# rjzhb/VectorSearch-RBAC

Hardware: AMD Instinct MI355X
Metric: QPS at recall@100, SIFT10M filtered-kNN (role RBAC), 1/2/4/8 MI355X (higher is better)
Workload: dtype int8 planes -> i32 (exact: bit-identical to the fp32 distances of vector.c)

## Files before the change

vectorsearch-rbac_amd/csrc/vsr_device.h:

```cpp
#pragma once
#include <hip/hip_runtime.h>
#include <stdint.h>
#include "vsr_bounds.h"

namespace vsr {

using f32x4 = __attribute__((ext_vector_type(4))) float;
using u32x4 = __attribute__((ext_vector_type(4))) uint32_t;
using i32x4 = __attribute__((ext_vector_type(4))) int;
using bf16x8 = __attribute__((ext_vector_type(8))) __bf16;
using f16x8 = __attribute__((ext_vector_type(8))) _Float16;

#ifdef __HIPCC__
template <class T> using gptr = const __attribute__((address_space(1))) T*;
template <class T> __device__ __forceinline__ gptr<T> as_global(const T* p) { return (gptr<T>) p; }
template <class T> __device__ __forceinline__ T lds_peek(const T* p)
{
    return *(const volatile __attribute__((address_space(3))) T*) p;
}
__device__ __forceinline__ uint2 load_tile(gptr<uint2> tiles, uint32_t t)
{
    const uint64_t v = ((gptr<uint64_t>) tiles)[t];
    return make_uint2((uint32_t) v, (uint32_t) (v >> 32));
}
#endif

constexpr uint64_t KEY_EMPTY = ~0ull;
constexpr int      SCAN_THREADS = 512;
constexpr int      SCAN_WAVES = SCAN_THREADS / 64;
constexpr int      SELECT_THREADS = 1024;
constexpr int      MAX_K = 2048;
constexpr int      SCAN_QMAX = 16;
constexpr size_t   SCAN_LDS_BUDGET = 72 * 1024;

constexpr int scan_slack(int rw) { return SCAN_WAVES * rw > 256 ? SCAN_WAVES * rw : 256; }

enum Metric : int { M_L2 = 0, M_IP = 1, M_COSINE = 2, M_L1 = 3 };

struct ScanGroup {
    const uint2*    tiles;
    const uint64_t* bitmap;
    uint32_t        n_tiles;
    uint32_t        q_begin;
    uint32_t        q_count;
    uint32_t        block_begin;
    uint32_t        n_blocks;
    uint32_t        partial_begin;
};

struct FusedTail {
    uint32_t        enable;
    uint32_t        fan;
    ScanGroup       group;
    uint32_t*       done;
    const int64_t*  block_ids;
    const int32_t*  doc_ids;
    const int64_t*  orig_rows;
    int64_t*        out_block;
    int32_t*        out_doc;
    int64_t*        out_row;
    float*          out_dist;
    uint64_t*       out_keys;
    int32_t*        out_count;
    int32_t*        out_flag;
    int32_t*        flag_total;
    uint32_t        row_offset;
    int             metric;
    uint64_t*       dbg;
};

#ifndef VSR_MW_DENSE
#define VSR_MW_DENSE 1
#endif

struct ScanParams {
    const float4*    rows;
    const float*     norm2;
    uint32_t         n_rows;
    uint32_t         stride4;
    const float*     queries;
    const float*     q_norm2;
    const ScanGroup* groups;
    uint32_t         n_groups;
    const uint32_t*  q_slots;
    uint64_t*        partial;
    uint32_t         kp;
    uint32_t         k;
    uint32_t         cap;
    uint32_t         qmax;
    uint64_t*        cand;
    uint32_t         rw;
    const uint64_t*  tau_init;
    uint32_t         sample_stride;
    const uint2*     block_map;
    const uint4*     scr;
    const uint4*     q_scr;
    uint32_t         pstride4;
    const uint4*     scr_c;
    const uint4*     q_scr_c;
    uint32_t         cstride4;
    uint32_t         plane_ho;
    uint64_t*        qcand;
    uint32_t*        qcnt;
    uint32_t         capq;
    const uint32_t*  rank;
    const uint64_t*  ones;
// ... 280 lines not shown
```

vectorsearch-rbac_amd/csrc/vsr_i8r.h:

```cpp
#pragma once
#include <type_traits>
#include "vsr_device.h"
#include "vsr_topk.h"
#include "vsr_mfma.h"

namespace vsr {

constexpr int KR_THREADS = 256;
constexpr int KR_WAVES = 4;
constexpr int KR_RING = 4;
constexpr int KR_OCC = 5;

template <int NQG>
__global__ __launch_bounds__(KR_THREADS, KR_OCC) void i8_sample_reg_kernel(const ScanParams p)
{
    constexpr int NC = NQG * 16;
    static_assert(NC == 64, "one lane of the appending wave per query column");
    __shared__ __align__(16) uint4 s_b[NQG * 2 * 64];
    __shared__ uint2 s_col[NC];
    static_assert(sizeof(uint4) * NQG * 2 * 64 >= sizeof(uint64_t) * KR_WAVES * NC * 4, "minima do not fit the B area");
    const int tid = threadIdx.x;
    const int lane = tid & 63;
    const int wave = __builtin_amdgcn_readfirstlane(tid >> 6);

    uint32_t lo = 0, hi = p.n_groups;
    while (hi - lo > 1) {
        const uint32_t mid = (lo + hi) >> 1;
        if (p.groups[mid].block_begin <= blockIdx.x) lo = mid; else hi = mid;
    }
    const ScanGroup grp = p.groups[lo];
    const uint32_t local_block = blockIdx.x - grp.block_begin;
    const auto g_tiles = as_global(grp.tiles);
    const auto g_norm2 = as_global(p.norm2);
    const auto g_rank = as_global(p.rank);
    const uint32_t q_count = grp.q_count;

    uint4 bq[2];
#pragma unroll
    for (int e = 0; e < 2; ++e) {
        const uint32_t idx = (uint32_t) tid + 256u * e;
        const uint32_t qi = (idx >> 7) * 16u + (idx & 15u);
        const uint32_t slot = p.q_slots[grp.q_begin + (qi < q_count ? qi : 0u)];
        bq[e] = p.q_scr[(size_t) slot * p.pstride4 + ((idx >> 6) & 1u) * 4u + ((idx & 63u) >> 4)];
    }
    if (tid < NC) {
        const bool qok = (uint32_t) tid < q_count;
        const uint32_t slot = p.q_slots[grp.q_begin + (qok ? (uint32_t) tid : 0u)];
        s_col[tid] = make_uint2(__float_as_uint(p.q_norm2[slot]), qok ? slot : 0xFFFFFFFFu);
    }

    const uint32_t t0 = (uint32_t) (((uint64_t) grp.n_tiles * local_block) / grp.n_blocks);
    const uint32_t t1 = (uint32_t) (((uint64_t) grp.n_tiles * (local_block + 1)) / grp.n_blocks);
    const uint32_t ss = p.sample_stride;
    const uint32_t n_st = (((t1 - t0 + 1u) >> 1) + ss - 1u) / ss;
    const uint32_t n_w = n_st > (uint32_t) wave ? (n_st - (uint32_t) wave + 3u) >> 2 : 0u;
    const uint32_t n_units = 2u * n_w;
    const uint32_t unit_last = n_units ? n_units - 1u : 0u;

    const uint32_t tile_last = grp.n_tiles - 1u;
    uint32_t row_lo, row_hi;
    bool bad_row;
    {
        const uint2 da = load_tile(g_tiles, t0 < tile_last ? t0 : tile_last);
        const uint2 db = load_tile(g_tiles, t1 > t0 && t1 - 1u < tile_last ? t1 - 1u : tile_last);
        row_lo = (uint32_t) __builtin_amdgcn_readfirstlane((int) da.x);
        row_hi = t1 > t0 ? (uint32_t) __builtin_amdgcn_readfirstlane((int) (db.x + db.y)) : row_lo;
        bad_row = row_hi > p.n_rows || row_hi < row_lo;
        row_hi = bad_row ? row_lo : row_hi;
    }
    const uint32_t row_clamp = (p.n_rows - 1u) & ~15u;

    const int li = lane & 15;
    const int kq = lane >> 4;
    const uint32_t ngt = (q_count + 15u) >> 4;
    const uint32_t voff = (uint32_t) li * 128u + (uint32_t) kq * 16u;
    const char* scr = reinterpret_cast<const char*>(p.scr);

    auto unit_row = [&](uint32_t u) -> uint32_t {
        const uint32_t uc = u < unit_last ? u : unit_last;
        return row_lo + 32u * ss * ((uint32_t) wave + 4u * (uc >> 1)) + 16u * (uc & 1u);
    };
    i32x4 a8[KR_RING][2];
    f32x4 nrm[KR_RING];
    auto issue = [&](auto K, uint32_t u) {
        constexpr int k = decltype(K)::value;
        const uint32_t r0 = unit_row(u);
        const uint32_t rc = r0 < row_clamp ? r0 : row_clamp;
        const gptr<uint4> src = as_global(reinterpret_cast<const uint4*>(scr + (size_t) rc * 128u + voff));
        a8[k][0] = __builtin_bit_cast(i32x4, src[0]);
        a8[k][1] = __builtin_bit_cast(i32x4, src[4]);
        nrm[k] = *reinterpret_cast<gptr<f32x4>>(g_norm2 + rc + (uint32_t) kq * 4u);
    };
    issue(std::integral_constant<int, 0>{}, 0u);
    issue(std::integral_constant<int, 1>{}, 1u);
    issue(std::integral_constant<int, 2>{}, 2u);

    s_b[tid] = bq[0];
    s_b[tid + 256] = bq[1];
    asm volatile("s_waitcnt lgkmcnt(0)\n\ts_barrier" ::: "memory");

    int64_t smin[NQG];
#pragma unroll
    for (int j = 0; j < NQG; ++j) smin[j] = ((int64_t) 0x3FFFFFFF << 32);
    auto compute = [&](auto K, uint32_t u) {
        constexpr int k = decltype(K)::value;
        const uint32_t row = unit_row(u) + (uint32_t) kq * 4u;
        int32_t nx[4];
#pragma unroll
        for (int r = 0; r < 4; ++r) nx[r] = row + (uint32_t) r < row_hi ? (int32_t) nrm[k][r] : 0x3FFFFFFF;
#pragma unroll
        for (int j = 0; j < NQG; ++j) {
            if ((uint32_t) j < ngt) {
                const i32x4 b0 = __builtin_bit_cast(i32x4, s_b[(j * 2 + 0) * 64 + lane]);
                const i32x4 b1 = __builtin_bit_cast(i32x4, s_b[(j * 2 + 1) * 64 + lane]);
                i32x4 acc = i32x4{0, 0, 0, 0};
                acc = __builtin_amdgcn_mfma_i32_16x16x64_i8(a8[k][0], b0, acc, 0, 0, 0);
                acc = __builtin_amdgcn_mfma_i32_16x16x64_i8(a8[k][1], b1, acc, 0, 0, 0);
#pragma unroll
                for (int r = 0; r < 4; ++r) {
                    const int32_t w = nx[r] - 2 * acc[r];
                    const int64_t cand = ((int64_t) w << 32) | (int64_t) (row + (uint32_t) r);
                    smin[j] = cand < smin[j] ? cand : smin[j];
                }
            }
        }
    };
    for (uint32_t u = 0; u < n_units; u += 4u) {
        issue(std::integral_constant<int, 3>{}, u + 3u);
        compute(std::integral_constant<int, 0>{}, u);
        issue(std::integral_constant<int, 0>{}, u + 4u);
        compute(std::integral_constant<int, 1>{}, u + 1u);
        issue(std::integral_constant<int, 1>{}, u + 5u);
        compute(std::integral_constant<int, 2>{}, u + 2u);
        issue(std::integral_constant<int, 2>{}, u + 6u);
        compute(std::integral_constant<int, 3>{}, u + 3u);
    }

    asm volatile("s_waitcnt lgkmcnt(0)\n\ts_barrier" ::: "memory");
    uint64_t* keys = reinterpret_cast<uint64_t*>(s_b);
#pragma unroll
    for (int j = 0; j < NQG; ++j) {
        const int32_t w = (int32_t) (smin[j] >> 32);
        uint64_t key = KEY_EMPTY;
        if ((uint32_t) j < ngt && w < 0x20000000) {
            const uint2 cc = s_col[j * 16 + li];
            const uint32_t row = (uint32_t) smin[j];
            if (cc.y != 0xFFFFFFFFu) key = make_key((float) w + __uint_as_float(cc.x), g_rank ? g_rank[row] : row);
        }
        keys[(wave * NC + j * 16 + li) * 4 + kq] = key;
    }
    asm volatile("s_waitcnt lgkmcnt(0)\n\ts_barrier" ::: "memory");
    if (wave == 0) {
        const int c = lane;
        const uint32_t slot = s_col[c].y;
        uint64_t keys16[4 * KR_WAVES];
        uint32_t n = 0;
#pragma unroll
        for (int w2 = 0; w2 < KR_WAVES; ++w2)
#pragma unroll
            for (int q4 = 0; q4 < 4; ++q4) {
                const uint64_t kk = keys[(w2 * NC + c) * 4 + q4];
                keys16[w2 * 4 + q4] = kk;
                n += kk != KEY_EMPTY;
            }
        if (n && slot != 0xFFFFFFFFu) {
            uint32_t at = atomicAdd(p.qcnt + slot, n);
#pragma unroll
            for (int t = 0; t < 4 * KR_WAVES; ++t)
                if (keys16[t] != KEY_EMPTY) {
                    if (at < p.capq) p.qcand[(size_t) slot * p.capq + at] = keys16[t];
                    ++at;
                }
        }
// ... 13 lines not shown
```

vectorsearch-rbac_amd/csrc/vsr_mfmaw.h:

```cpp
#pragma once
#include <type_traits>
#include "vsr_device.h"
#include "vsr_scan.h"
#include "vsr_topk.h"
#include "vsr_mfma.h"
#include "vsr_i8s.h"
#include "vsr_i8r.h"

namespace vsr {

constexpr int MW_THREADS = 256;
constexpr int MW_WAVES = 4;
constexpr int MW_S = 16;
constexpr int MW_ROWS = 64;
constexpr int MW_NQ = MF_NQ * MW_WAVES;
constexpr int MW_RING = 8;

#ifndef VSR_MW_DEPTH1
#define VSR_MW_DEPTH1 1
#endif
#ifndef VSR_MW_OCC1
#define VSR_MW_OCC1 3
#endif
#ifndef VSR_ABLATE
// ... 130 lines not shown
    const uint32_t g1 = (uint32_t) wave + 4u;
    const bool gact2 = NG == 2 && rsplit == 1u && g1 < ngt;
    const uint32_t my_qi2 = g1 * MF_NQ + (uint32_t) jq;
    const bool qok2 = gact2 && my_qi2 < q_count;
    uint32_t my_slot2 = my_slot;
    float my_qn2 = 0.0f, tau_lim2 = -__builtin_inff();
    const uint4* my_qsrc2 = nullptr;
    bf16x8 bh2[NBLK], bm2[NBLK];
    if constexpr (NG == 2) {
        my_slot2 = p.q_slots[grp.q_begin + (qok2 ? my_qi2 : 0u)];
        const uint64_t t2 = p.tau_init ? p.tau_init[my_slot2] : KEY_EMPTY;
        tau_lim2 = t2 == KEY_EMPTY ? __builtin_inff() : mono_to_float((uint32_t) (t2 >> 32));
        my_qn2 = p.q_norm2[my_slot2];
        my_qsrc2 = p.q_scr + (size_t) my_slot2 * (HO ? 2 * pstride4 : pstride4);
#pragma unroll
        for (int blk = 0; blk < NBLK; ++blk) {
            bh2[blk] = __builtin_bit_cast(bf16x8, my_qsrc2[blk * 4 + kq]);
            bm2[blk] = __builtin_bit_cast(bf16x8, my_qsrc2[(HO ? 16 : 8) + blk * 4 + kq]);
        }
    }
    const uint32_t col_slot = lane < MF_NQ ? my_slot : my_slot2;

    const uint32_t tile_last = grp.n_tiles - 1u;
    auto fetch_desc = [&](uint32_t it_) -> uint2 {
        const uint32_t t = t0 + it_ * ss * tps + (uint32_t) lane / rw;
        const bool ok = it_ < n_it && t < t1;
        const uint2 d = load_tile(g_tiles, t < tile_last ? t : tile_last);
        return make_uint2(ok ? d.x : 0u, ok ? d.y : 0u);
    };
    int32_t  pend_row[DEPTH];
    uint64_t pend_bw[DEPTH];
    float    pend_nrm[DEPTH];
    uint2    dsc_a[DEPTH];
#pragma unroll
    for (int j = 0; j < DEPTH; ++j) {
        pend_row[j] = -1;
        pend_bw[j] = ~0ull;
        pend_nrm[j] = 0.0f;
        dsc_a[j] = make_uint2(0u, 0u);
    }
    bool bad_row = false;
    uint32_t row_lo = 0, row_hi = 0;
    if constexpr (DENSE) {
        const uint2 da = load_tile(g_tiles, t0 < tile_last ? t0 : tile_last);
        const uint2 db = load_tile(g_tiles, t1 > t0 && t1 - 1u < tile_last ? t1 - 1u : tile_last);
        row_lo = (uint32_t) __builtin_amdgcn_readfirstlane((int) da.x);
        row_hi = t1 > t0 ? (uint32_t) __builtin_amdgcn_readfirstlane((int) (db.x + db.y)) : row_lo;
        bad_row = row_hi > p.n_rows || row_hi < row_lo;
        row_hi = bad_row ? row_lo : row_hi;
    }
    auto start_dense = [&](uint32_t it_, int32_t& row, uint64_t& bw, float& nrm) {
        const uint32_t rr = row_lo + it_ * (uint32_t) MW_ROWS + (uint32_t) lane;
        const bool ok = it_ < n_it && rr < row_hi;
        row = ok ? (int32_t) rr : -1;
        bw = ~0ull;
        nrm = g_norm2[ok ? rr : 0u];
    };
    auto start_rows = [&](uint2 d, int32_t& row, uint64_t& bw, float& nrm) {
        const uint32_t r = (uint32_t) lane % rw;
        const uint32_t rr = d.x + r;
        const bool ok = r < d.y && rr < p.n_rows;
        bad_row |= r < d.y && rr >= p.n_rows;
        const uint32_t rc = ok ? rr : 0u;
        row = ok ? (int32_t) rr : -1;
        bw = *(g_bitmap ? g_bitmap + (rc >> 6) : g_ones);
        nrm = g_norm2[rc];
    };
    auto finish_rows = [&](uint32_t it_, int32_t row, uint64_t bw, float nrm) {
        if (row >= 0 && !((bw >> ((uint32_t) row & 63u)) & 1ull)) row = -1;
        if (wave == 0) {
            rowidx[(it_ % MW_RING) * 64 + lane] = row;
            rownorm[(it_ % MW_RING) * 64 + lane] = row >= 0 ? nrm : __builtin_nanf("");
            if constexpr (ITEST) rowthr[(it_ % MW_RING) * 64 + lane] = row >= 0 ? ((int32_t) nrm) >> 1 : 0x7FFFFFFF;
        }
    };
    if constexpr (DENSE) {
#pragma unroll
        for (int j = 0; j < DEPTH; ++j) {
            int32_t r0;
            uint64_t b0;
            float n0;
            start_dense((uint32_t) j, r0, b0, n0);
            finish_rows((uint32_t) j, r0, b0, n0);
            start_dense((uint32_t) (DEPTH + j), pend_row[j], pend_bw[j], pend_nrm[j]);
        }
    } else {
        uint2 d[2 * DEPTH];
#pragma unroll
        for (int j = 0; j < 2 * DEPTH; ++j) d[j] = fetch_desc((uint32_t) j);
#pragma unroll
        for (int j = 0; j < DEPTH; ++j) dsc_a[j] = fetch_desc((uint32_t) (2 * DEPTH + j));
#pragma unroll
        for (int j = 0; j < DEPTH; ++j) {
            int32_t r0;
            uint64_t b0;
            float n0;
            start_rows(d[j], r0, b0, n0);
            finish_rows((uint32_t) j, r0, b0, n0);
            start_rows(d[DEPTH + j], pend_row[j], pend_bw[j], pend_nrm[j]);
        }
    }
    __syncthreads();

    const int lrow = I8 ? tid >> 3 : tid >> 4, lchunk = I8 ? tid & 7 : tid & 15;
    constexpr int LROWS = I8 ? 32 : 16;
    uint4 X[DEPTH][NCHR][NU];
    const uint32_t last_row = p.n_rows - 1u;
    auto issue = [&](auto dc, auto sc, uint32_t it_) {
        constexpr int D = decltype(dc)::value;
        constexpr int S = decltype(sc)::value;
        const uint32_t chunk = (uint32_t) (S * SR + lchunk);
        const int32_t* ridx = rowidx + (it_ % MW_RING) * 64;
#pragma unroll
        for (int u = 0; u < NU; ++u) {
            uint32_t rc;
            if constexpr (DENSE) {
                const uint32_t rr = row_lo + it_ * (uint32_t) MW_ROWS + (uint32_t) (u * LROWS + lrow);
                rc = it_ < n_it && rr < row_hi ? rr : 0u;
            } else {
                const int32_t r = ridx[u * LROWS + lrow];
                rc = (uint32_t) (r < 0 ? 0 : r);
            }
            if ((VSR_ABLATE & 8) && it_ > 0) continue;
            const u32x4 v = *reinterpret_cast<const u32x4*>(p.scr + (size_t) (rc < last_row ? rc : last_row) * pstride4 + chunk);
            X[D][S][u] = make_uint4(v[0], v[1], v[2], v[3]);
        }
    };
    const uint32_t nch_rt = LONG ? pstride4 / (uint32_t) SR : (uint32_t) NCH;
    auto issue_rt = [&](uint32_t it_, uint32_t s_) {
        const uint32_t chunk = s_ * (uint32_t) SR + (uint32_t) lchunk;
        const int32_t* ridx = rowidx + (it_ % MW_RING) * 64;
#pragma unroll
        for (int u = 0; u < NU; ++u) {
            const int32_t r = ridx[u * LROWS + lrow];
            const uint32_t rc = (uint32_t) (r < 0 ? 0 : r);
            const u32x4 v = *reinterpret_cast<const u32x4*>(p.scr + (size_t) (rc < last_row ? rc : last_row) * pstride4 + chunk);
            X[0][0][u] = make_uint4(v[0], v[1], v[2], v[3]);
        }
    };
    auto load_b = [&](uint32_t s_, bf16x8 (&h)[NBLK], bf16x8 (&m)[NBLK]) {
#pragma unroll
        for (int blk = 0; blk < NBLK; ++blk) {
            h[blk] = __builtin_bit_cast(bf16x8, my_qsrc[s_ * (HO ? 32u : 16u) + (uint32_t) (blk * 4 + kq)]);
            m[blk] = __builtin_bit_cast(bf16x8, my_qsrc[s_ * (HO ? 32u : 16u) + (HO ? 16u : 8u) + (uint32_t) (blk * 4 + kq)]);
        }
    };
    auto issue_tile = [&](auto dc, uint32_t it_) {
        if constexpr (LONG) {
            issue_rt(it_, 0u);
            return;
        }
        issue(dc, std::integral_constant<int, 0>{}, it_);
        if constexpr (NCH > 1) issue(dc, std::integral_constant<int, 1>{}, it_);
        if constexpr (NCH > 2) issue(dc, std::integral_constant<int, 2>{}, it_);
    };
    const uint32_t n_pad = (n_it + DEPTH - 1) / DEPTH * DEPTH;
    issue_tile(std::integral_constant<int, 0>{}, 0);
    if constexpr (DEPTH > 1) issue_tile(std::integral_constant<int, 1>{}, 1);
    if constexpr (DEPTH > 2) issue_tile(std::integral_constant<int, 2>{}, 2);
    if constexpr (DEPTH > 3) issue_tile(std::integral_constant<int, 3>{}, 3);

    uint32_t p_head = 0, p_tail = 0, f_n = 0;
    constexpr int FL_R = 2;
    uint32_t f_rank[FL_R];
    uint32_t f_base = 0;
#pragma unroll
    for (int r = 0; r < FL_R; ++r) f_rank[r] = 0;
    auto flush_issue = [&]() __attribute__((always_inline)) {
        const uint32_t have = p_tail - p_head;
        f_n = have < 64u * FL_R ? have : 64u * FL_R;
        uint32_t col[FL_R];
#pragma unroll
        for (int r = 0; r < FL_R; ++r) {
            const uint32_t e = (uint32_t) (r * 64 + lane);
            col[r] = e < f_n ? pend_c[(p_head + e) % MW_PEND] : 0xFFu;
        }
        uint32_t mine = 0;
#pragma unroll
        for (int c = 0; c < MF_NQ * NG; ++c) {
            uint32_t before = 0;
#pragma unroll
            for (int r = 0; r < FL_R; ++r) {
                const uint64_t m = __ballot(col[r] == (uint32_t) c);
                if (col[r] == (uint32_t) c)
                    f_rank[r] = before + __builtin_amdgcn_mbcnt_hi((uint32_t) (m >> 32), __builtin_amdgcn_mbcnt_lo((uint32_t) m, 0u));
                before += (uint32_t) __popcll(m);
            }
            if (lane == c) mine = before;
        }
        if (lane < MF_NQ * NG && mine) f_base = atomicAdd(p.qcnt + col_slot, mine);
    };
    auto flush_store = [&]() __attribute__((always_inline)) {
#pragma unroll
        for (int r = 0; r < FL_R; ++r) {
            const uint32_t e = (uint32_t) (r * 64 + lane);
            const uint32_t idx = (p_head + e) % MW_PEND;
            const uint32_t c = e < f_n ? pend_c[idx] : 0u;
            const uint32_t base = (uint32_t) __shfl((int) f_base, (int) c);
            const uint32_t slot = (uint32_t) __shfl((int) col_slot, (int) c);
            if (e < f_n) {
                const uint32_t row = pend_r[idx];
                const uint32_t at = base + f_rank[r];
                if (at < p.capq)
                    p.qcand[(size_t) slot * p.capq + at] = ((uint64_t) pend_v[idx] << 32) | (g_rank ? g_rank[row] : row);
            }
        }
        p_head += f_n;
        f_n = 0;
    };
    auto park_mask = [&](uint64_t act, bool has, uint32_t key_hi, uint32_t row, uint32_t col = 0xFFFFFFFFu, uint32_t slot_ = 0u)
                         __attribute__((always_inline)) {
        if (col == 0xFFFFFFFFu) {
            col = (uint32_t) jq;
            slot_ = my_slot;
        }
        const uint32_t room = MW_PEND - (p_tail - p_head);
        const uint32_t rank = __builtin_amdgcn_mbcnt_hi((uint32_t) (act >> 32), __builtin_amdgcn_mbcnt_lo((uint32_t) act, 0u));
        if (has) {
            if (rank < room) {
                const uint32_t at = (p_tail + rank) % MW_PEND;
                pend_v[at] = key_hi;
                pend_r[at] = row;
                pend_c[at] = col;
            } else {
                const uint32_t ga = atomicAdd(p.qcnt + slot_, 1u);
                if (ga < p.capq) p.qcand[(size_t) slot_ * p.capq + ga] = ((uint64_t) key_hi << 32) | (g_rank ? g_rank[row] : row);
            }
        }
        const uint32_t n_act = (uint32_t) __popcll(act);
        p_tail += n_act < room ? n_act : room;
    };
    auto park = [&](bool has, uint32_t key_hi, uint32_t row, uint32_t col = 0xFFFFFFFFu, uint32_t slot_ = 0u)
                    __attribute__((always_inline)) {
        park_mask(__ballot(has), has, key_hi, row, col, slot_);
    };

    auto run = [&](auto nsc) {
        constexpr int NS = decltype(nsc)::value;
        constexpr int NH = NS > 2 ? 2 : NS;
        int buf = 0;
        auto tile = [&](auto dc, uint32_t it) {
            constexpr int D = decltype(dc)::value;
            f32x4 acc[NS];
            f32x4 acc2[NS];
            i32x4 acc8[NS];
#pragma unroll
            for (int i = 0; i < NS; ++i) {
                acc[i] = f32x4{0.f, 0.f, 0.f, 0.f};
                acc2[i] = f32x4{0.f, 0.f, 0.f, 0.f};
                acc8[i] = ITEST ? i32x4{c0, c0, c0, c0} : i32x4{0, 0, 0, 0};
            }

            auto do_stage = [&](auto sc) {
                constexpr int S = decltype(sc)::value;
                uint4* img = stage + (size_t) buf * (MW_ROWS * SR);
#pragma unroll
                for (int u = 0; u < NU; ++u) {
                    const int slot = u * LROWS + lrow;
                    img[slot * SR + (lchunk ^ (slot & (SR - 1)))] = X[D][S][u];
                }
                if constexpr (S == 0) {
                    if (f_n) flush_store();
                    finish_rows(it + DEPTH, pend_row[D], pend_bw[D], pend_nrm[D]);
                    if constexpr (DENSE) start_dense(it + 2 * DEPTH, pend_row[D], pend_bw[D], pend_nrm[D]);
                    else {
                        start_rows(dsc_a[D], pend_row[D], pend_bw[D], pend_nrm[D]);
                        dsc_a[D] = fetch_desc(it + 3 * DEPTH);
                    }
                }
                lds_barrier();
                if constexpr (S == 0) {
                    if (!f_n && p_tail - p_head >= 64u * FL_R) flush_issue();
                }
                issue(dc, sc, it + DEPTH);
                if constexpr (I8) {
                    if (gact && !(VSR_ABLATE & 4)) {
#pragma unroll
                        for (int blk = 0; blk < NBLK; ++blk) {
                            i32x4 a8[NS];
#pragma unroll
                            for (int i = 0; i < NS; ++i) {
                                const int row = ((int) sub0 + i) * 16 + li;
                                a8[i] = __builtin_bit_cast(i32x4, img[row * SR + ((blk * 4 + kq) ^ (row & (SR - 1)))]);
                            }
#pragma unroll
                            for (int i = 0; i < NS; ++i) acc8[i] = __builtin_amdgcn_mfma_i32_16x16x64_i8(a8[i], b8[blk], acc8[i], 0, 0, 0);
                        }
                    }
                } else if (gact && !(VSR_ABLATE & 4)) {
#pragma unroll
                    for (int h0 = 0; h0 < NS; h0 += NH)
#pragma unroll
                        for (int blk = 0; blk < NBLK; ++blk) {
                            bf16x8 ah[NH], am[NH];
#pragma unroll
                            for (int i = 0; i < NH; ++i) {
                                const int row = ((int) sub0 + h0 + i) * 16 + li;
                                ah[i] = __builtin_bit_cast(bf16x8, img[row * MW_S + ((blk * 4 + kq) ^ li)]);
                                if constexpr (!HO) am[i] = __builtin_bit_cast(bf16x8, img[row * MW_S + ((8 + blk * 4 + kq) ^ li)]);
                            }
#pragma unroll
                            for (int i = 0; i < NH; ++i) acc[h0 + i] = __builtin_amdgcn_mfma_f32_16x16x32_bf16(ah[i], bh[S][blk], acc[h0 + i], 0, 0, 0);
#pragma unroll
                            for (int i = 0; i < NH; ++i) acc[h0 + i] = __builtin_amdgcn_mfma_f32_16x16x32_bf16(ah[i], bm[S][blk], acc[h0 + i], 0, 0, 0);
                            if constexpr (!HO) {
#pragma unroll
                                for (int i = 0; i < NH; ++i) acc[h0 + i] = __builtin_amdgcn_mfma_f32_16x16x32_bf16(am[i], bh[S][blk], acc[h0 + i], 0, 0, 0);
                            }
                        }
                }
                buf ^= 1;
            };
            if constexpr (LONG) {
                for (uint32_t s = 0; s < nch_rt; ++s) {
                    uint4* img = stage + (size_t) buf * (MW_ROWS * SR);
#pragma unroll
                    for (int u = 0; u < NU; ++u) {
                        const int slot = u * LROWS + lrow;
                        img[slot * SR + (lchunk ^ (slot & (SR - 1)))] = X[0][0][u];
                    }
                    {
#if VSR_LONG_MAP_EVERY_STAGE
                        int32_t r2;
                        uint64_t b2;
                        float n2;
                        start_rows(dsc_a[0], r2, b2, n2);
                        const uint2 d2 = fetch_desc(it + 3);
                        if (s == 0) {
                            if (f_n) flush_store();
                            finish_rows(it + 1, pend_row[0], pend_bw[0], pend_nrm[0]);
                            pend_row[0] = r2;
                            pend_bw[0] = b2;
                            pend_nrm[0] = n2;
                            dsc_a[0] = d2;
                        }
#else
                        if (s == 0) {
                            if (f_n) flush_store();
                            finish_rows(it + 1, pend_row[0], pend_bw[0], pend_nrm[0]);
                            start_rows(dsc_a[0], pend_row[0], pend_bw[0], pend_nrm[0]);
                            dsc_a[0] = fetch_desc(it + 3);
                        }
#endif
                    }
                    lds_barrier();
                    if (s == 0 && !f_n && p_tail - p_head >= 64u * FL_R) flush_issue();
                    const bool last = s + 1 == nch_rt;
                    issue_rt(last ? it + 1 : it, last ? 0u : s + 1);
                    bf16x8 nh[NBLK], nm[NBLK], nh2[NBLK], nm2[NBLK];
                    load_b(last ? 0u : s + 1, nh, nm);
                    if constexpr (NG == 2) {
                        const uint32_t sn = last ? 0u : s + 1;
#pragma unroll
                        for (int blk = 0; blk < NBLK; ++blk) {
                            nh2[blk] = __builtin_bit_cast(bf16x8, my_qsrc2[sn * (HO ? 32u : 16u) + (uint32_t) (blk * 4 + kq)]);
                            nm2[blk] = __builtin_bit_cast(bf16x8, my_qsrc2[sn * (HO ? 32u : 16u) + (HO ? 16u : 8u) + (uint32_t) (blk * 4 + kq)]);
                        }
// ... 258 lines not shown
```

vectorsearch-rbac_amd/csrc/vsr_scan.h:

```cpp
#pragma once
#include "vsr_device.h"
#include "vsr_topk.h"

namespace vsr {

template <int V> struct Log2 { static constexpr int value = 1 + Log2<V / 2>::value; };
template <> struct Log2<1> { static constexpr int value = 0; };

template <int METRIC>
__device__ __forceinline__ void accum4(float& p, const float4& x, const float4& q)
{
    if constexpr (METRIC == M_L2) {
        const float d0 = x.x - q.x, d1 = x.y - q.y, d2 = x.z - q.z, d3 = x.w - q.w;
        p = fmaf(d0, d0, p); p = fmaf(d1, d1, p); p = fmaf(d2, d2, p); p = fmaf(d3, d3, p);
    } else if constexpr (METRIC == M_L1) {
        p += fabsf(x.x - q.x); p += fabsf(x.y - q.y); p += fabsf(x.z - q.z); p += fabsf(x.w - q.w);
    } else {
        p = fmaf(x.x, q.x, p); p = fmaf(x.y, q.y, p); p = fmaf(x.z, q.z, p); p = fmaf(x.w, q.w, p);
    }
}

__device__ __forceinline__ void widen8(const uint4& h, float4& a, float4& b)
{
    const f16x8 v = __builtin_bit_cast(f16x8, h);
// ... 197 lines not shown
    }
    return cnt[1];
}

__device__ __forceinline__ void fused_tail(const ScanParams& p, const ScanGroup& grp, uint32_t local_block, uint64_t* keys,
                                        int tid, bool bad = false, uint64_t t_start = 0, uint64_t t_scan = 0, uint64_t t_pub = 0)
{
    __shared__ uint32_t s_last;
    const FusedTail& f = p.fused;
    uint64_t t_m1 = 0, t_m1s = 0;
    const uint32_t B = grp.n_blocks, fan = f.fan, n_g = (B + fan - 1) / fan, k = p.k, kp = p.kp;
    const uint32_t my_g = local_block / fan;
    const uint32_t g_size = (my_g + 1) * fan <= B ? fan : B - my_g * fan;
    uint64_t* lists = p.partial + (size_t) grp.partial_begin * kp;
    __syncthreads();
    if (tid == 0) s_last = atomicAdd(f.done + 1 + my_g, 1u) == g_size - 1u;
    __syncthreads();
    if (!s_last) return;
    const uint64_t* src = lists;
    uint32_t n_src = B * kp;
    if (n_g > 1) {
        if (f.dbg) t_m1s = wall_clock64();
        const uint32_t n = fused_block_select(lists + (size_t) my_g * fan * kp, g_size * kp, k, keys, tid);
        if (f.dbg) t_m1 = wall_clock64();
        uint64_t* dst = lists + (size_t) (B + my_g) * kp;
        for (uint32_t i = tid; i < kp; i += SCAN_THREADS)
            __hip_atomic_store(dst + i, i < n ? keys[i] : KEY_EMPTY, __ATOMIC_RELAXED, __HIP_MEMORY_SCOPE_AGENT);
        __syncthreads();
        if (tid == 0) s_last = atomicAdd(f.done, 1u) == n_g - 1u;
        __syncthreads();
        if (!s_last) return;
        src = lists + (size_t) B * kp;
        n_src = n_g * kp;
    }
    const uint64_t t_m2s = f.dbg ? wall_clock64() : 0;
    const uint32_t m = fused_block_select(src, n_src, k, keys, tid);
    const uint64_t t_m2 = f.dbg ? wall_clock64() : 0;
    for (uint32_t i = tid; i < k; i += SCAN_THREADS) {
        if (i < m) {
            const uint64_t key = keys[i];
            uint32_t at = 0;
            for (uint32_t j = 0; j < m; ++j) at += keys[j] < key;
            const uint32_t row = (uint32_t) key;
            const float v = mono_to_float((uint32_t) (key >> 32));
            f.out_block[at] = f.block_ids[row];
            f.out_doc[at] = f.doc_ids[row];
            if (f.out_row) f.out_row[at] = f.orig_rows[row];
            f.out_dist[at] = f.metric == M_L2 ? (float) sqrt((double) v) : v;
            if (f.out_keys) f.out_keys[at] = (key & 0xFFFFFFFF00000000ull) | (uint64_t) (row + f.row_offset);
        } else {
            f.out_block[i] = -1;
            f.out_doc[i] = -1;
            if (f.out_row) f.out_row[i] = -1;
            f.out_dist[i] = __builtin_inff();
            if (f.out_keys) f.out_keys[i] = KEY_EMPTY;
        }
    }
    if (tid == 0) {
        f.out_count[0] = bad ? -1 - (int32_t) m : (int32_t) m;
        f.out_flag[0] = bad ? 1 : 0;
        if (bad && f.flag_total) atomicAdd(f.flag_total, 1);
    }
    for (uint32_t i = tid; i < 1 + n_g; i += SCAN_THREADS) f.done[i] = 0;
    if (f.dbg && tid == 0) {
        f.dbg[0] = t_start; f.dbg[1] = t_scan; f.dbg[2] = t_pub; f.dbg[3] = t_m1s; f.dbg[4] = t_m1; f.dbg[5] = t_m2s; f.dbg[6] = t_m2;
        f.dbg[7] = wall_clock64();
    }
}

#ifndef VSR_PREFETCH
#define VSR_PREFETCH 0
#endif
#ifndef VSR_MINWAVES
#define VSR_MINWAVES 2
#endif

template <int METRIC, int LPR, int C, int R, int QI, bool HALF = false>
__global__ __launch_bounds__(SCAN_THREADS, (HALF && QI == 1 ? 4 : VSR_MINWAVES)) void scan_kernel(const ScanParams p)
{
    using S = ScanShape<LPR, R>;
    constexpr int G = S::G, RW = S::RW, D = S::D, XCHK = S::XCHK;
    constexpr int CC = C > 0 ? C : 1;
    using Chunk = typename std::conditional<HALF, uint4, float4>::type;

    extern __shared__ __align__(16) unsigned char smem[];
    const int tid = threadIdx.x;
    const int lane = tid & 63;
    const int wave = __builtin_amdgcn_readfirstlane(tid >> 6);
    const int l = lane % LPR;
    const int g = lane / LPR;

    const bool fused = QI == 1 && p.fused.enable;
    uint32_t lo = 0, hi = fused ? 1u : p.n_groups;
    while (hi - lo > 1) {
        const uint32_t mid = (lo + hi) >> 1;
        if (p.groups[mid].block_begin <= blockIdx.x) lo = mid; else hi = mid;
    }
    const ScanGroup grp = fused ? p.fused.group : p.groups[lo];
    const auto g_tiles = as_global(grp.tiles);
    const auto g_bitmap = as_global(grp.bitmap);
    const auto g_rank = as_global(p.rank);
    const uint32_t local_block = blockIdx.x - grp.block_begin;
    const uint32_t t0 = (uint32_t) (((uint64_t) grp.n_tiles * local_block) / grp.n_blocks);
    const uint32_t t1 = (uint32_t) (((uint64_t) grp.n_tiles * (local_block + 1)) / grp.n_blocks);

    const uint32_t cap = p.cap, k = p.k, qmax = p.qmax, stride4 = p.stride4;
    const uint32_t rstride = HALF ? stride4 / 2 : stride4;
    uint64_t* keys = reinterpret_cast<uint64_t*>(smem);
    TopKCtrl* ctrl = reinterpret_cast<TopKCtrl*>(keys + (size_t) qmax * cap);
    float4*   qlds = reinterpret_cast<float4*>(ctrl + qmax);
    float*    qnl = reinterpret_cast<float*>(qlds + (size_t) qmax * stride4);
    uint32_t* flags = reinterpret_cast<uint32_t*>(qnl + qmax);

    const uint32_t q_count = grp.q_count;
    const uint32_t n_sub = (q_count + QI - 1) / QI;
    for (uint32_t qi = tid; qi < qmax; qi += SCAN_THREADS) {
        const uint32_t slot = fused ? 0u : p.q_slots[grp.q_begin + (qi < q_count ? qi : 0)];
        ctrl[qi].tau = p.tau_init ? p.tau_init[slot] : KEY_EMPTY;
        ctrl[qi].count = 0;
        qnl[qi] = (METRIC == M_COSINE) ? p.q_norm2[slot] : 0.0f;
    }
    if (tid < 4) flags[tid] = 0;
    for (uint32_t qi = 0; qi < n_sub * QI; ++qi) {
        const uint32_t slot = fused ? 0u : p.q_slots[grp.q_begin + (qi < q_count ? qi : 0)];
        const float4* qsrc = reinterpret_cast<const float4*>(p.queries) + (size_t) slot * stride4;
        for (uint32_t i = tid; i < stride4; i += SCAN_THREADS)
            qlds[(size_t) qi * stride4 + i] = HALF ? round_to_half(qsrc[i]) : qsrc[i];
    }
    __syncthreads();

    const bool own = (l % D) == 0;
    const int row_own = (l / D) * G + g;
    const uint32_t trigger = cap - S::SLACK;
    const uint32_t ss = p.sample_stride;
    const uint32_t iters = ((t1 - t0 + ss - 1) / ss + SCAN_WAVES - 1) / SCAN_WAVES;

    auto fetch = [&](uint32_t t, TileRegs<R, CC, Chunk>& tr) {
        tr.mask = 0;
        tr.start = 0;
        tr.rn = 0.0f;
        if (t >= t1) return;
        uint32_t start, nrows;
        if (g_tiles) {
            const uint2 tl = load_tile(g_tiles, t);
            start = tl.x;
            nrows = tl.y;
        } else {
            start = t * RW;
            nrows = p.n_rows - start < (uint32_t) RW ? p.n_rows - start : (uint32_t) RW;
        }
        uint64_t mask = nrows >= 64 ? ~0ull : ((1ull << nrows) - 1ull);
        if (g_bitmap) mask &= bitmap_window(g_bitmap, start);
        tr.start = start;
        tr.mask = mask;
        if (!mask) return;
        if constexpr (METRIC == M_COSINE) {
            if (own && ((mask >> row_own) & 1ull)) tr.rn = p.norm2[start + row_own];
        }
        if constexpr (C > 0) {
            const Chunk* base = reinterpret_cast<const Chunk*>(p.rows) + (size_t) start * rstride;
#pragma unroll
            for (int r = 0; r < R; ++r) {
                const int row = r * G + g;
                const bool ok = (mask >> row) & 1ull;
#pragma unroll
                for (int c = 0; c < C; ++c) {
                    const uint32_t chunk = c * LPR + l;
                    tr.x[r][c] = (ok && chunk < rstride) ? base[(size_t) row * rstride + chunk] : zero_chunk<Chunk>();
                }
            }
        }
    };

    TileRegs<R, CC, Chunk> cur;
#if VSR_PREFETCH
    TileRegs<R, CC, Chunk> nxt;
    fetch(t0 + wave * ss, cur);
#endif
    uint32_t round = 0;
    for (uint32_t it = 0; it < iters; ++it) {
#if VSR_PREFETCH
        if (it + 1 < iters) fetch(t0 + ((it + 1) * SCAN_WAVES + wave) * ss, nxt);
        else nxt.mask = 0;
#else
        fetch(t0 + (it * SCAN_WAVES + wave) * ss, cur);
#endif

        if (cur.mask) {
            const uint32_t start = cur.start;
            const bool ok_own = (cur.mask >> row_own) & 1ull;
            if constexpr (C > 0) {
                for (uint32_t sb = 0; sb < n_sub; ++sb) {
                    float acc[QI][R];
#pragma unroll
                    for (int qi = 0; qi < QI; ++qi)
#pragma unroll
                        for (int r = 0; r < R; ++r) acc[qi][r] = 0.0f;
#pragma unroll
                    for (int c = 0; c < C; ++c) {
                        const uint32_t chunk = c * LPR + l;
                        if constexpr (HALF) {
                            float4 qa[QI], qb[QI];
#pragma unroll
                            for (int qi = 0; qi < QI; ++qi) {
                                const float4* qrow = qlds + (size_t) (sb * QI + qi) * stride4 + 2 * chunk;
                                qa[qi] = chunk < rstride ? qrow[0] : make_float4(0.f, 0.f, 0.f, 0.f);
                                qb[qi] = chunk < rstride ? qrow[1] : make_float4(0.f, 0.f, 0.f, 0.f);
                            }
#pragma unroll
                            for (int r = 0; r < R; ++r) {
                                float4 xa, xb;
                                widen8(cur.x[r][c], xa, xb);
#pragma unroll
                                for (int qi = 0; qi < QI; ++qi) {
                                    accum4<METRIC>(acc[qi][r], xa, qa[qi]);
                                    accum4<METRIC>(acc[qi][r], xb, qb[qi]);
                                }
                            }
                        } else {
#pragma unroll
                            for (int qi = 0; qi < QI; ++qi) {
                                const float4 qv = chunk < stride4 ? qlds[(size_t) (sb * QI + qi) * stride4 + chunk]
                                                                  : make_float4(0.f, 0.f, 0.f, 0.f);
#pragma unroll
                                for (int r = 0; r < R; ++r) accum4<METRIC>(acc[qi][r], cur.x[r][c], qv);
                            }
                        }
                    }
#pragma unroll
                    for (int qi = 0; qi < QI; ++qi) {
                        const uint32_t qs = sb * QI + qi;
                        reduce_slots<LPR / 2, R>(acc[qi], lane);
                        const float v = rank_value<METRIC>(acc[qi][0], cur.rn, qnl[qs]);
                        const uint64_t key = make_key(v, g_rank ? g_rank[start + row_own] : start + row_own);
                        const uint64_t tau = lds_peek(&ctrl[qs].tau);
                        const bool pass = own && ok_own && qs < q_count && key < tau;
                        topk_append(keys + (size_t) qs * cap, &ctrl[qs], pass, key);
                    }
                }
            } else {
                const Chunk* base = reinterpret_cast<const Chunk*>(p.rows) + (size_t) start * rstride;
                float acc[QI][R];
#pragma unroll
                for (int qi = 0; qi < QI; ++qi)
#pragma unroll
                    for (int r = 0; r < R; ++r) acc[qi][r] = 0.0f;
#pragma unroll 4
                for (uint32_t chunk = l; chunk < rstride; chunk += 64) {
                    Chunk x[R];
#pragma unroll
                    for (int r = 0; r < R; ++r) {
                        const bool ok = (cur.mask >> r) & 1ull;
                        x[r] = ok ? base[(size_t) r * rstride + chunk] : zero_chunk<Chunk>();
                    }
                    if constexpr (HALF) {
                        float4 qa[QI], qb[QI];
#pragma unroll
                        for (int qi = 0; qi < QI; ++qi) {
                            const float4* qrow = qlds + (size_t) qi * stride4 + 2 * chunk;
                            qa[qi] = qrow[0];
                            qb[qi] = qrow[1];
                        }
#pragma unroll
                        for (int r = 0; r < R; ++r) {
                            float4 xa, xb;
                            widen8(x[r], xa, xb);
#pragma unroll
                            for (int qi = 0; qi < QI; ++qi) {
                                accum4<METRIC>(acc[qi][r], xa, qa[qi]);
                                accum4<METRIC>(acc[qi][r], xb, qb[qi]);
                            }
                        }
                    } else {
#pragma unroll
                        for (int qi = 0; qi < QI; ++qi) {
                            const float4 qv = qlds[(size_t) qi * stride4 + chunk];
#pragma unroll
                            for (int r = 0; r < R; ++r) accum4<METRIC>(acc[qi][r], x[r], qv);
                        }
                    }
                }
#pragma unroll
                for (int qi = 0; qi < QI; ++qi) {
                    reduce_slots<LPR / 2, R>(acc[qi], lane);
                    const float v = rank_value<METRIC>(acc[qi][0], cur.rn, qnl[qi]);
                    const uint64_t key = make_key(v, g_rank ? g_rank[start + row_own] : start + row_own);
                    const uint64_t tau = lds_peek(&ctrl[qi].tau);
                    const bool pass = own && ok_own && (uint32_t) qi < q_count && key < tau;
                    topk_append(keys + (size_t) qi * cap, &ctrl[qi], pass, key);
                }
            }
        }

        if ((it % XCHK) == XCHK - 1 && it + 1 < iters) {
            bool need = false;
            for (uint32_t qs = 0; qs < q_count; ++qs)
                need |= lds_peek(&ctrl[qs].count) > trigger;
            const uint32_t slot = round % 3;
            if (need && lane == 0) atomicOr(&flags[slot], 1u);
            __syncthreads();
            const bool any = lds_peek(&flags[slot]) != 0;
            if (tid == 0) flags[(round + 2) % 3] = 0;
            ++round;
            if (any) {
                for (uint32_t qs = 0; qs < q_count; ++qs)
                    if (ctrl[qs].count > trigger)
                        topk_compact<SCAN_THREADS>(keys + (size_t) qs * cap, &ctrl[qs], k, tid, false);
            }
        }
#if VSR_PREFETCH
        cur = nxt;
#endif
    }

    __syncthreads();
    for (uint32_t qs = 0; qs < q_count; ++qs) {
        uint32_t n;
        if (fused && ctrl[qs].count <= (uint32_t) (SCAN_THREADS * FUSED_KPT)) {
            const uint32_t have = ctrl[qs].count;
            n = have > k ? fused_block_select<true>(keys, have, k, keys, tid) : have;
        } else {
            topk_compact<SCAN_THREADS>(keys + (size_t) qs * cap, &ctrl[qs], k, tid, false);
            n = ctrl[qs].count < k ? ctrl[qs].count : k;
        }
        uint64_t* dst = p.partial + (size_t) (grp.partial_begin + qs * grp.n_blocks + local_block) * p.kp;
        if (fused) {
            for (uint32_t i = tid; i < p.kp; i += SCAN_THREADS)
                __hip_atomic_store(dst + i, i < n ? keys[(size_t) qs * cap + i] : KEY_EMPTY, __ATOMIC_RELAXED,
                                   __HIP_MEMORY_SCOPE_AGENT);
        } else {
            for (uint32_t i = tid; i < p.kp; i += SCAN_THREADS) dst[i] = i < n ? keys[(size_t) qs * cap + i] : KEY_EMPTY;
        }
    }
    if constexpr (QI == 1) {
        if (fused) fused_tail(p, grp, local_block, keys, tid);
    }
// ... 43 lines not shown
```

vectorsearch-rbac_amd/csrc/vsr_scan8.h:

```cpp
#pragma once
#include "vsr_scan.h"

namespace vsr {

#ifndef SCAN8_DEPTH
#define SCAN8_DEPTH 4
#endif

__global__ __launch_bounds__(SCAN_THREADS, 2) void scan8_fused_kernel(const ScanParams p, uint32_t dim, uint32_t* q8_bad_host)
{
    constexpr int RW = 16, XCHK = scan_slack(RW) / (SCAN_WAVES * RW);
    static_assert(XCHK >= 1, "append slack");
    const uint64_t t_start = p.fused.dbg ? wall_clock64() : 0;
    extern __shared__ __align__(16) unsigned char smem[];
    const int tid = threadIdx.x;
    const int lane = tid & 63;
    const int wave = __builtin_amdgcn_readfirstlane(tid >> 6);
    const int l = lane & 7;
    const int g = lane >> 3;
    const ScanGroup grp = p.fused.group;
    const auto g_tiles = as_global(grp.tiles);
    const auto g_bitmap = as_global(grp.bitmap);
    const uint32_t local_block = blockIdx.x;
    const uint32_t t0 = (uint32_t) (((uint64_t) grp.n_tiles * local_block) / grp.n_blocks);
    const uint32_t t1 = (uint32_t) (((uint64_t) grp.n_tiles * (local_block + 1)) / grp.n_blocks);
    const uint32_t cap = p.cap, k = p.k;
    uint64_t* keys = reinterpret_cast<uint64_t*>(smem);
    TopKCtrl* ctrl = reinterpret_cast<TopKCtrl*>(keys + cap);
    uint32_t* q8 = reinterpret_cast<uint32_t*>(ctrl + 1);
    uint32_t* flags = q8 + 32;
    const uint32_t trigger = cap - (uint32_t) scan_slack(RW);
    const uint32_t iters = ((t1 - t0) + SCAN_WAVES - 1) / SCAN_WAVES;
    const uint32_t last_row = p.n_rows - 1u;

    constexpr int DEPTH = SCAN8_DEPTH;
    struct Tile { uint4 x[2]; float rn[2]; };
    uint32_t round = 0;
    uint32_t d_start = 0, d_mask = 0;
    uint32_t nj = 0;
    auto load_desc = [&](uint32_t cb) {
        const uint32_t t = t0 + (cb + (uint32_t) lane) * SCAN_WAVES + (uint32_t) wave;
        const bool have = cb + (uint32_t) lane < iters && t < t1;
        const uint32_t tc = have ? t : t0;
        uint2 tl = make_uint2(0u, 0u);
        if (g_tiles) {
            if (t0 < t1) tl = load_tile(g_tiles, tc);
        } else {
            tl.x = tc * RW;
            tl.y = p.n_rows - tl.x < (uint32_t) RW ? p.n_rows - tl.x : (uint32_t) RW;
        }
        uint32_t mask = tl.y >= 16u ? 0xFFFFu : (1u << tl.y) - 1u;
        if (g_bitmap) mask &= (uint32_t) bitmap_window(g_bitmap, tl.x);
        d_start = tl.x;
        d_mask = have ? mask : 0u;
        nj = iters - cb < 64u ? iters - cb : 64u;
    };
    auto fetch = [&](uint32_t j, Tile& tr, uint32_t& start, uint32_t& mask) {
        const uint32_t jc = j < nj ? j : 0u;
        start = (uint32_t) __builtin_amdgcn_readlane((int) d_start, (int) jc);
        mask = j < nj ? (uint32_t) __builtin_amdgcn_readlane((int) d_mask, (int) jc) : 0u;
#pragma unroll
        for (int r = 0; r < 2; ++r) {
            const uint32_t row = start + (uint32_t) (r * 8 + g);
            const bool ok = (mask >> (r * 8 + g)) & 1u;
            const uint32_t rc = ok && row <= last_row ? row : (start <= last_row ? start : last_row);
            tr.x[r] = p.scr[(size_t) rc * 8 + l];
            tr.rn[r] = p.norm2[rc];
        }
    };
    Tile ring[DEPTH];
    uint32_t r_start[DEPTH], r_mask[DEPTH];
    float xs[4];
#pragma unroll
    for (int e = 0; e < 4; ++e) {
        const uint32_t j = (uint32_t) (tid & 31) * 4 + (uint32_t) e;
        xs[e] = p.queries[j < dim ? j : 0u];
    }
    load_desc(0);
#pragma unroll
    for (int d = 0; d < DEPTH; ++d) fetch((uint32_t) d, ring[d], r_start[d], r_mask[d]);

    if (tid == 0) {
        ctrl[0].tau = KEY_EMPTY;
        ctrl[0].count = 0;
    }
    if (tid < 8) flags[tid] = 0;
    __syncthreads();
    if (tid < 32) {
        uint32_t word = 0, n2 = 0;
        bool bad = false;
#pragma unroll
        for (int e = 0; e < 4; ++e) {
            const uint32_t j = (uint32_t) tid * 4 + (uint32_t) e;
            int b = 0;
            if (j < dim) {
                const float x = xs[e];
                bad |= !(x >= 0.0f && x <= 255.0f && x == floorf(x));
                b = (int) fminf(fmaxf(x, 0.0f), 255.0f) - 128;
                n2 += (uint32_t) (b * b);
            }
            word |= ((uint32_t) b & 0xFFu) << (8 * e);
        }
        q8[tid] = word;
        atomicAdd(&flags[5], n2);
        if (bad) flags[4] = 1u;
    }
    __syncthreads();
    const bool bad_query = lds_peek(&flags[4]) != 0;
    const float qn = (float) lds_peek(&flags[5]);
    const int4 qv = *reinterpret_cast<const int4*>(q8 + l * 4);
    for (uint32_t cb = 0; cb < iters; cb += 64) {
        if (cb) {
            load_desc(cb);
#pragma unroll
            for (int d = 0; d < DEPTH; ++d) fetch((uint32_t) d, ring[d], r_start[d], r_mask[d]);
        }
        for (uint32_t j0 = 0; j0 < nj; j0 += DEPTH) {
#pragma unroll
            for (int d = 0; d < DEPTH; ++d) {
                const uint32_t j = j0 + (uint32_t) d, it = cb + j;
                const Tile cur = ring[d];
                const uint32_t c_start = r_start[d], c_mask = r_mask[d];
                fetch(j + DEPTH, ring[d], r_start[d], r_mask[d]);
                if (c_mask) {
#pragma unroll
                    for (int r = 0; r < 2; ++r) {
                        int dot = 0;
                        dot = __builtin_amdgcn_sdot4((int) cur.x[r].x, qv.x, dot, false);
                        dot = __builtin_amdgcn_sdot4((int) cur.x[r].y, qv.y, dot, false);
                        dot = __builtin_amdgcn_sdot4((int) cur.x[r].z, qv.z, dot, false);
                        dot = __builtin_amdgcn_sdot4((int) cur.x[r].w, qv.w, dot, false);
                        dot += __shfl_xor(dot, 1);
                        dot += __shfl_xor(dot, 2);
                        dot += __shfl_xor(dot, 4);
                        const uint32_t row = c_start + (uint32_t) (r * 8 + g);
                        const bool ok = l == 0 && ((c_mask >> (r * 8 + g)) & 1u);
                        const float v = fmaf(-2.0f, (float) dot, cur.rn[r] + qn);
                        const uint64_t key = make_key(v, row);
                        const bool pass = ok && key < lds_peek(&ctrl[0].tau);
                        topk_append(keys, &ctrl[0], pass, key);
                    }
                }
                if (j < nj && (it % XCHK) == XCHK - 1 && it + 1 < iters) {
                    const bool need = lds_peek(&ctrl[0].count) > trigger;
                    const uint32_t slot = round % 3;
                    if (need && lane == 0) atomicOr(&flags[slot], 1u);
                    __syncthreads();
                    const bool any = lds_peek(&flags[slot]) != 0;
                    if (tid == 0) flags[(round + 2) % 3] = 0;
// ... 37 lines not shown
```

Baseline: 3.767 million.

## Use nontemporal loads for streamed rows and defer dense row prefetch issue

Adds a compile-time VSR_STREAM_NT mask that routes the streaming 16-byte row loads in several scan kernels through nontemporal loads. The default mask only enables this for the single-query scan8 and scan paths (STREAM_K1). It also reorders the dense MFMA-wide kernel so finish_rows/start_dense for the next ring slot happen after issuing the current tile rather than before, with the initial start_dense calls moved after the prologue. The aim is to reduce cache pollution from one-pass data and improve load overlap, at the cost of possible changes in L2 reuse and register pressure.

```diff
diff --git a/vectorsearch-rbac_amd/csrc/vsr_device.h b/vectorsearch-rbac_amd/csrc/vsr_device.h
--- a/vectorsearch-rbac_amd/csrc/vsr_device.h
+++ b/vectorsearch-rbac_amd/csrc/vsr_device.h
@@ -22,6 +22,24 @@
 {
     const uint64_t v = ((gptr<uint64_t>) tiles)[t];
     return make_uint2((uint32_t) v, (uint32_t) (v >> 32));
+}
+#endif
+
+#ifndef VSR_STREAM_NT
+#define VSR_STREAM_NT 4
+#endif
+constexpr int STREAM_K2W = 1, STREAM_K2R = 2, STREAM_K1 = 4;
+
+#ifdef __HIPCC__
+template <class T> __device__ __forceinline__ T load_stream16(gptr<T> p)
+{
+    static_assert(sizeof(T) == 16, "one dwordx4");
+    return __builtin_bit_cast(T, __builtin_nontemporal_load((gptr<u32x4>) p));
+}
+template <int BIT, class T> __device__ __forceinline__ T load_row16(const T* p)
+{
+    if constexpr ((VSR_STREAM_NT & BIT) != 0) return load_stream16(as_global(p));
+    else return *p;
 }
 #endif
 
diff --git a/vectorsearch-rbac_amd/csrc/vsr_i8r.h b/vectorsearch-rbac_amd/csrc/vsr_i8r.h
--- a/vectorsearch-rbac_amd/csrc/vsr_i8r.h
+++ b/vectorsearch-rbac_amd/csrc/vsr_i8r.h
@@ -87,8 +87,13 @@
         const uint32_t r0 = unit_row(u);
         const uint32_t rc = r0 < row_clamp ? r0 : row_clamp;
         const gptr<uint4> src = as_global(reinterpret_cast<const uint4*>(scr + (size_t) rc * 128u + voff));
-        a8[k][0] = __builtin_bit_cast(i32x4, src[0]);
-        a8[k][1] = __builtin_bit_cast(i32x4, src[4]);
+        if constexpr ((VSR_STREAM_NT & STREAM_K2R) != 0) {
+            a8[k][0] = __builtin_bit_cast(i32x4, load_stream16(src));
+            a8[k][1] = __builtin_bit_cast(i32x4, load_stream16(src + 4));
+        } else {
+            a8[k][0] = __builtin_bit_cast(i32x4, src[0]);
+            a8[k][1] = __builtin_bit_cast(i32x4, src[4]);
+        }
         nrm[k] = *reinterpret_cast<gptr<f32x4>>(g_norm2 + rc + (uint32_t) kq * 4u);
     };
     issue(std::integral_constant<int, 0>{}, 0u);
diff --git a/vectorsearch-rbac_amd/csrc/vsr_mfmaw.h b/vectorsearch-rbac_amd/csrc/vsr_mfmaw.h
--- a/vectorsearch-rbac_amd/csrc/vsr_mfmaw.h
+++ b/vectorsearch-rbac_amd/csrc/vsr_mfmaw.h
@@ -236,7 +236,6 @@
             float n0;
             start_dense((uint32_t) j, r0, b0, n0);
             finish_rows((uint32_t) j, r0, b0, n0);
-            start_dense((uint32_t) (DEPTH + j), pend_row[j], pend_bw[j], pend_nrm[j]);
         }
     } else {
         uint2 d[2 * DEPTH];
@@ -276,7 +275,7 @@
                 rc = (uint32_t) (r < 0 ? 0 : r);
             }
             if ((VSR_ABLATE & 8) && it_ > 0) continue;
-            const u32x4 v = *reinterpret_cast<const u32x4*>(p.scr + (size_t) (rc < last_row ? rc : last_row) * pstride4 + chunk);
+            const u32x4 v = load_row16<STREAM_K2W>(reinterpret_cast<const u32x4*>(p.scr + (size_t) (rc < last_row ? rc : last_row) * pstride4 + chunk));
             X[D][S][u] = make_uint4(v[0], v[1], v[2], v[3]);
         }
     };
@@ -288,7 +287,7 @@
         for (int u = 0; u < NU; ++u) {
             const int32_t r = ridx[u * LROWS + lrow];
             const uint32_t rc = (uint32_t) (r < 0 ? 0 : r);
-            const u32x4 v = *reinterpret_cast<const u32x4*>(p.scr + (size_t) (rc < last_row ? rc : last_row) * pstride4 + chunk);
+            const u32x4 v = load_row16<STREAM_K2W>(reinterpret_cast<const u32x4*>(p.scr + (size_t) (rc < last_row ? rc : last_row) * pstride4 + chunk));
             X[0][0][u] = make_uint4(v[0], v[1], v[2], v[3]);
         }
     };
@@ -313,6 +312,10 @@
     if constexpr (DEPTH > 1) issue_tile(std::integral_constant<int, 1>{}, 1);
     if constexpr (DEPTH > 2) issue_tile(std::integral_constant<int, 2>{}, 2);
     if constexpr (DEPTH > 3) issue_tile(std::integral_constant<int, 3>{}, 3);
+    if constexpr (DENSE) {
+#pragma unroll
+        for (int j = 0; j < DEPTH; ++j) start_dense((uint32_t) (DEPTH + j), pend_row[j], pend_bw[j], pend_nrm[j]);
+    }
 
     uint32_t p_head = 0, p_tail = 0, f_n = 0;
     constexpr int FL_R = 2;
@@ -415,9 +418,8 @@
                 }
                 if constexpr (S == 0) {
                     if (f_n) flush_store();
-                    finish_rows(it + DEPTH, pend_row[D], pend_bw[D], pend_nrm[D]);
-                    if constexpr (DENSE) start_dense(it + 2 * DEPTH, pend_row[D], pend_bw[D], pend_nrm[D]);
-                    else {
+                    if constexpr (!DENSE) {
+                        finish_rows(it + DEPTH, pend_row[D], pend_bw[D], pend_nrm[D]);
                         start_rows(dsc_a[D], pend_row[D], pend_bw[D], pend_nrm[D]);
                         dsc_a[D] = fetch_desc(it + 3 * DEPTH);
                     }
@@ -427,6 +429,10 @@
                     if (!f_n && p_tail - p_head >= 64u * FL_R) flush_issue();
                 }
                 issue(dc, sc, it + DEPTH);
+                if constexpr (S == 0 && DENSE) {
+                    finish_rows(it + DEPTH, pend_row[D], pend_bw[D], pend_nrm[D]);
+                    start_dense(it + 2 * DEPTH, pend_row[D], pend_bw[D], pend_nrm[D]);
+                }
                 if constexpr (I8) {
                     if (gact && !(VSR_ABLATE & 4)) {
 #pragma unroll
diff --git a/vectorsearch-rbac_amd/csrc/vsr_scan.h b/vectorsearch-rbac_amd/csrc/vsr_scan.h
--- a/vectorsearch-rbac_amd/csrc/vsr_scan.h
+++ b/vectorsearch-rbac_amd/csrc/vsr_scan.h
@@ -303,6 +303,7 @@
     constexpr int G = S::G, RW = S::RW, D = S::D, XCHK = S::XCHK;
     constexpr int CC = C > 0 ? C : 1;
     using Chunk = typename std::conditional<HALF, uint4, float4>::type;
+    constexpr int NTB = QI == 1 ? STREAM_K1 : 0;
 
     extern __shared__ __align__(16) unsigned char smem[];
     const int tid = threadIdx.x;
@@ -387,7 +388,10 @@
 #pragma unroll
                 for (int c = 0; c < C; ++c) {
                     const uint32_t chunk = c * LPR + l;
-                    tr.x[r][c] = (ok && chunk < rstride) ? base[(size_t) row * rstride + chunk] : zero_chunk<Chunk>();
+                    if constexpr ((VSR_STREAM_NT & NTB) != 0)
+                        tr.x[r][c] = (ok && chunk < rstride) ? load_stream16(as_global(base + (size_t) row * rstride + chunk)) : zero_chunk<Chunk>();
+                    else
+                        tr.x[r][c] = (ok && chunk < rstride) ? base[(size_t) row * rstride + chunk] : zero_chunk<Chunk>();
                 }
             }
         }
@@ -472,7 +476,8 @@
 #pragma unroll
                     for (int r = 0; r < R; ++r) {
                         const bool ok = (cur.mask >> r) & 1ull;
-                        x[r] = ok ? base[(size_t) r * rstride + chunk] : zero_chunk<Chunk>();
+                        if constexpr ((VSR_STREAM_NT & NTB) != 0) x[r] = ok ? load_stream16(as_global(base + (size_t) r * rstride + chunk)) : zero_chunk<Chunk>();
+                        else x[r] = ok ? base[(size_t) r * rstride + chunk] : zero_chunk<Chunk>();
                     }
                     if constexpr (HALF) {
                         float4 qa[QI], qb[QI];
diff --git a/vectorsearch-rbac_amd/csrc/vsr_scan8.h b/vectorsearch-rbac_amd/csrc/vsr_scan8.h
--- a/vectorsearch-rbac_amd/csrc/vsr_scan8.h
+++ b/vectorsearch-rbac_amd/csrc/vsr_scan8.h
@@ -64,7 +64,7 @@
             const uint32_t row = start + (uint32_t) (r * 8 + g);
             const bool ok = (mask >> (r * 8 + g)) & 1u;
             const uint32_t rc = ok && row <= last_row ? row : (start <= last_row ? start : last_row);
-            tr.x[r] = p.scr[(size_t) rc * 8 + l];
+            tr.x[r] = load_row16<STREAM_K1>(p.scr + (size_t) rc * 8 + l);
             tr.rn[r] = p.norm2[rc];
         }
     };
```

After: 3.791 million, median of 2. About the same (+0.6%).
